# Tanveer81/ReVisionLLM

Measured on AMD Instinct MI355X. Metric: video-segments/sec (whole node), stage-2 100-seg recursion, Vicuna-7B, higher is better.
Workload: dtype fp16

## Files before the change

### revisionllm_amd/csrc/gemm_pp.hip

```cpp
#include <algorithm>
#include <atomic>
#include <type_traits>

#include "kernels.h"

#ifndef PP_ABL
#define PP_ABL 0
#endif
#if PP_ABL & 32
__device__ __attribute__((visibility("default"))) unsigned long long pp_stamp_buf[256 * 2 * 9];
__device__ __attribute__((visibility("default"))) unsigned long long pp_stamp_ext[3 * 256 * 4];
#endif

namespace {

typedef const __attribute__((address_space(1))) void* gptr_t;
typedef __attribute__((address_space(3))) void* lptr_t;
__device__ __forceinline__ void glds16(const void* g, void* l) { __builtin_amdgcn_global_load_lds((gptr_t)g, (lptr_t)l, 16, 0, 0); }
__device__ __forceinline__ float silu(float x) { return rv_silu(x); }

constexpr int PBM = 256, PBN = 256, PBK = 64;
constexpr int UNIT = 128 * 128;
constexpr int PP_LDS = 10 * UNIT;

// ... 24 lines not shown
#pragma unroll
    for (int i = 0; i < 2; ++i) {
        const int lr = (wave * 2 + i) * 8 + (lane >> 3);
        const int chunk = (lane & 7) ^ (lane >> 3);
        const int trow = (lr >> 6) * 128 + (lr & 63);
        int g0 = m0 + trow, g1 = m0 + trow + 64;
        g0 = g0 < M ? g0 : M - 1;
        g1 = g1 < M ? g1 : M - 1;
        s.a0[i] = (unsigned)(((int64_t)g0 * lda + chunk * 8) * 2);
        s.a1[i] = (unsigned)(((int64_t)g1 * lda + chunk * 8) * 2);
    }
    const int kfr = K >> 5;
    const int nb0 = ((PP_ABL & 16) ? 0 : (n0 >> 4)) + (wave >> 1) * NF + (wave & 1);
#pragma unroll
    for (int ks = 0; ks < 2; ++ks) {
        s.w0[ks] = (unsigned)(((((int64_t)nb0 * kfr + ks) * 64 + lane) * 8) * 2);
        s.w1[ks] = (unsigned)(((((int64_t)(nb0 + 2) * kfr + ks) * 64 + lane) * 8) * 2);
    }
    if constexpr (NF == 3) {
        const int nb1 = (n0 >> 4) + (wave >> 1) * NF + 2;
        s.w1[0] = (unsigned)(((((int64_t)nb1 * kfr + (wave & 1)) * 64 + lane) * 8) * 2);
    }
}

template <int U, int NF>
__device__ __forceinline__ void issue_unit(const PpSrc& s, int k0, char* dst0, int wave) {
    char* dst = dst0 + wave * 2048;
    const char* ab = s.A + (int64_t)k0 * 2;
    const char* wb = s.W + (int64_t)k0 * 32;
    if constexpr (U == 0) {
        glds16(ab + s.a0[0], dst);
        glds16(ab + s.a0[1], dst + 1024);
    } else if constexpr (U == 3) {
        glds16(ab + s.a1[0], dst);
        glds16(ab + s.a1[1], dst + 1024);
    } else if constexpr (U == 1) {
        glds16(wb + s.w0[0], dst);
        glds16(wb + s.w0[1], dst + 1024);
    } else if constexpr (NF == 4) {
        glds16(wb + s.w1[0], dst);
        glds16(wb + s.w1[1], dst + 1024);
    } else {
        glds16(wb + s.w1[0], dst0 + wave * 1024);
    }
}

template <int N_>
__device__ __forceinline__ void wait_vm() {
    static_assert(N_ >= 0 && N_ <= 14, "extend the table");
    if constexpr (N_ == 14) asm volatile("s_waitcnt vmcnt(14)" ::: "memory");
    else if constexpr (N_ == 13) asm volatile("s_waitcnt vmcnt(13)" ::: "memory");
    else if constexpr (N_ == 12) asm volatile("s_waitcnt vmcnt(12)" ::: "memory");
    else if constexpr (N_ == 11) asm volatile("s_waitcnt vmcnt(11)" ::: "memory");
    else if constexpr (N_ == 10) asm volatile("s_waitcnt vmcnt(10)" ::: "memory");
    else if constexpr (N_ == 9) asm volatile("s_waitcnt vmcnt(9)" ::: "memory");
    else if constexpr (N_ == 8) asm volatile("s_waitcnt vmcnt(8)" ::: "memory");
    else if constexpr (N_ == 7) asm volatile("s_waitcnt vmcnt(7)" ::: "memory");
    else if constexpr (N_ == 6) asm volatile("s_waitcnt vmcnt(6)" ::: "memory");
    else if constexpr (N_ == 5) asm volatile("s_waitcnt vmcnt(5)" ::: "memory");
    else if constexpr (N_ == 4) asm volatile("s_waitcnt vmcnt(4)" ::: "memory");
    else if constexpr (N_ == 3) asm volatile("s_waitcnt vmcnt(3)" ::: "memory");
    else if constexpr (N_ == 2) asm volatile("s_waitcnt vmcnt(2)" ::: "memory");
    else if constexpr (N_ == 1) asm volatile("s_waitcnt vmcnt(1)" ::: "memory");
    else asm volatile("s_waitcnt vmcnt(0)" ::: "memory");
}

#ifndef PP_ISSUE_MID
#define PP_ISSUE_MID 0
#endif
#ifndef PP_PRIO_MODE
#define PP_PRIO_MODE 1
#endif
#define _PP_C ,
constexpr int PP_A_STAGE = 2 * UNIT, PP_W_BASE = 2 * PP_A_STAGE, PP_W_STAGE = 2 * UNIT;
typedef int pp_i32x8 __attribute__((ext_vector_type(8)));
__device__ __forceinline__ pp_i32x8 pp_cat(op16x8 lo, op16x8 hi) {
    typedef int i32x4_ __attribute__((ext_vector_type(4)));
    const i32x4_ a = __builtin_bit_cast(i32x4_, lo), b = __builtin_bit_cast(i32x4_, hi);
    return pp_i32x8{a[0], a[1], a[2], a[3], b[0], b[1], b[2], b[3]};
}
#ifndef PP_KSPLIT
#define PP_KSPLIT 1
#endif
#ifndef PP_EARLY
#define PP_EARLY 0
#endif
__device__ __forceinline__ void glds16_sv(const char* sbase, unsigned voff, char* lds_dst) {
    const unsigned l = (unsigned)(uintptr_t)(lptr_t)lds_dst;
    asm volatile("s_mov_b32 m0, %2\n\ts_nop 0\n\tglobal_load_lds_dwordx4 %0, %1" : : "v"(voff), "s"(sbase), "s"(l) : "memory");
}
template <int KIND>
__device__ __forceinline__ void issue_ks(const PpSrc& s, int kt, char* dst0, int wave) {
    char* dst = dst0 + wave * 2048;
    const char* ab = s.A + (int64_t)kt * (PBK * 2);
    const char* wb = s.W + (int64_t)kt * (PBK * 32);
    if constexpr (KIND == 0) {
        glds16_sv(ab, s.a0[0], dst);
        glds16_sv(ab, s.a0[1], dst + 1024);
    } else if constexpr (KIND == 1) {
        glds16_sv(ab, s.a1[0], dst);
        glds16_sv(ab, s.a1[1], dst + 1024);
    } else {
        glds16_sv(wb, s.w0[KIND - 2], dst);
        glds16_sv(wb, s.w1[KIND - 2], dst + 1024);
    }
}
__device__ __forceinline__ void ks_issue_prologue(const PpSrc& src, int kt0, int nks, char* smem, int wave) {
    issue_ks<2>(src, kt0, smem + 1 * UNIT, wave);
    issue_ks<0>(src, kt0, smem + 2 * UNIT, wave);
    issue_ks<3>(src, kt0, smem + 3 * UNIT, wave);
    issue_ks<1>(src, kt0, smem + 4 * UNIT, wave);
    if (nks > 1) {
        issue_ks<2>(src, kt0 + 1, smem + 5 * UNIT, wave);
        issue_ks<0>(src, kt0 + 1, smem + 6 * UNIT, wave);
        issue_ks<3>(src, kt0 + 1, smem + 7 * UNIT, wave);
        issue_ks<1>(src, kt0 + 1, smem + 8 * UNIT, wave);
        if (nks > 2) issue_ks<2>(src, kt0 + 2, smem + 9 * UNIT, wave);
    }
}
template <int DUMMY = 0>
__device__ __forceinline__ void pp_mainloop_ks(f32x4 (&acc)[4][8], const PpSrc& src, int kt0, int nks, char* smem, int wave, int lane, [[maybe_unused]] int kind = 1,
                                               bool pre = false) {
    const int wr = wave >> 2, wc = wave & 3;
    const int fr = lane & 15, kg = lane >> 4;
    const int a_rd = (wr * 64 + fr) * 128;
    const int a_c0 = ((kg ^ (fr & 7)) << 4), a_c1 = (((4 + kg) ^ (fr & 7)) << 4);
    const int w_rd = wc * 4096 + lane * 16;
    auto slot = [&](int ib, int k) { const int x = ib + k; return smem + (x >= 10 ? x - 10 : x) * UNIT; };
    op16x8 A0[4], A1[4], W0[4], W1[4];
    [[maybe_unused]] uint32_t st_sum[8] = {0, 0, 0, 0, 0, 0, 0, 0};
    [[maybe_unused]] uint64_t st_prev = 0;
#if PP_ABL & 32
#define PP_STAMP(i) { const uint64_t t_ = __builtin_readcyclecounter(); st_sum[i] += (uint32_t)(t_ - st_prev); st_prev = t_; }
#else
#define PP_STAMP(i)
#endif
#define KS_READ_A(DST, BASE, CH)                                                                            \
    if constexpr (!(PP_ABL & 2)) _Pragma("unroll") for (int f = 0; f < 4; ++f) DST[f] = *(const op16x8*)((BASE) + a_rd + f * 2048 + (CH));
#define KS_READ_W(DST, BASE)                                                                                \
    if constexpr (!(PP_ABL & 2)) _Pragma("unroll") for (int j = 0; j < 4; ++j) DST[j] = *(const op16x8*)((BASE) + w_rd + (j & 1) * 2048 + (j >> 1) * 1024);
#define KS_MFMA(WB, AB, MI0)                                                                                \
    if constexpr (!(PP_ABL & 8)) _Pragma("unroll") for (int j = 0; j < 4; ++j) _Pragma("unroll") for (int f = 0; f < 4; ++f) \
        acc[j][(MI0) + f] = rv_mfma16(WB[j], AB[f], acc[j][(MI0) + f]);
#define KS_SYNC_M(WAITN)                                   \
    if constexpr (grp == 1) { WAITN; }                     \
    __builtin_amdgcn_sched_barrier(0);                     \
    if constexpr (!(PP_ABL & 4)) __builtin_amdgcn_s_barrier(); \
    __builtin_amdgcn_sched_barrier(0);
#define KS_SYNC_C(WAITN)                                   \
    __builtin_amdgcn_sched_barrier(0);                     \
    if constexpr (grp == 0) { WAITN; }                     \
    __builtin_amdgcn_sched_barrier(0);                     \
    if constexpr (!(PP_ABL & 4)) __builtin_amdgcn_s_barrier(); \
    __builtin_amdgcn_sched_barrier(0);
    if constexpr (PP_ABL & 2) {
        asm volatile("" : "=v"(A0[0]), "=v"(A0[1]), "=v"(A0[2]), "=v"(A0[3]), "=v"(A1[0]), "=v"(A1[1]), "=v"(A1[2]), "=v"(A1[3]));
        asm volatile("" : "=v"(W0[0]), "=v"(W0[1]), "=v"(W0[2]), "=v"(W0[3]), "=v"(W1[0]), "=v"(W1[1]), "=v"(W1[2]), "=v"(W1[3]));
    }

#if PP_ABL & 32
    const uint64_t t_in = __builtin_readcyclecounter();
#endif
    if (!pre) ks_issue_prologue(src, kt0, nks, smem, wave);
    if (nks > 2) wait_vm<14>();
    else if (nks > 1) wait_vm<12>();
    else wait_vm<4>();
    __builtin_amdgcn_s_barrier();
    KS_READ_A(A0, smem + 2 * UNIT, a_c0)
    KS_READ_W(W0, smem + 1 * UNIT)
    if (nks > 2) wait_vm<12>();
    else if (nks > 1) wait_vm<10>();
    else wait_vm<2>();
// ... 251 lines not shown
        s.a[i] = (unsigned)(((int64_t)g * lda + (((lane & 7) ^ (lane >> 3)) * 8)) * 2);
        const int nb = (n0 >> 4) + wave * 4 + (i >> 1);
        s.w[i] = (unsigned)(((((int64_t)nb * kfr + (i & 1)) * 64 + lane) * 8) * 2);
    }
}
constexpr int PP4_TILE = 256 * 64 * 2;
template <int DUMMY = 0>
__device__ __forceinline__ void pp4_mainloop(f32x4 (&acc)[8][8], const Pp4Src& src, int kt0, int nks, char* smem, int wave, int lane) {
    const int wr = wave >> 1, wc = wave & 1;
    const int fr = lane & 15, kg = lane >> 4;
    const int a_rd = (wr * 128 + fr) * 128;
    const int a_c[2] = {((kg ^ (fr & 7)) << 4), (((4 + kg) ^ (fr & 7)) << 4)};
    const int w_rd = wc * 16384 + lane * 16;
    op16x8 fa[2][8], fw[2][8];
#define P4_A_STAGE(c) (smem + ((c) & 1) * PP4_TILE)
#define P4_W_STAGE(ws) (smem + (2 + (ws)) * PP4_TILE)
#define P4_ISSUE_A(KT, ST, i) glds16(src.A + (int64_t)(KT) * 128 + src.a[i], (ST) + (wave * 8 + (i)) * 1024)
#define P4_ISSUE_W(KT, ST, i) glds16(src.W + (int64_t)(KT) * 2048 + src.w[i], (ST) + (wave * 8 + (i)) * 1024)
#define P4_READ_A(B, ST, KS, f) fa[B][f] = *(const op16x8*)((ST) + a_rd + (f) * 2048 + a_c[KS])
#define P4_READ_W(B, ST, KS, j) fw[B][j] = *(const op16x8*)((ST) + w_rd + (j) * 2048 + (KS) * 1024)
#define P4_MFMA1(B, j, f) asm volatile(RV_MFMA16_ASM " %0, %1, %2, %0" : "+a"(acc[j][f]) : "v"(fw[B][j]), "v"(fa[B][f]));
#define P4_MFMA2(B, j, f) P4_MFMA1(B, j, f) P4_MFMA1(B, j, (f) + 1)
#define P4_PIN __builtin_amdgcn_sched_barrier(0);
    const int last = kt0 + nks - 1;
    auto kclamp = [&](int k) { return k < last ? k : last; };
#pragma unroll
    for (int i = 0; i < 8; ++i) P4_ISSUE_A(kt0, P4_A_STAGE(0), i);
#pragma unroll
    for (int i = 0; i < 8; ++i) P4_ISSUE_W(kt0, P4_W_STAGE(0), i);
#pragma unroll
    for (int i = 0; i < 8; ++i) P4_ISSUE_W(kclamp(kt0 + 1), P4_W_STAGE(1), i);
#pragma unroll
    for (int i = 0; i < 8; ++i) P4_ISSUE_A(kclamp(kt0 + 1), P4_A_STAGE(1), i);
#pragma unroll
    for (int i = 0; i < 8; ++i) P4_ISSUE_W(kclamp(kt0 + 2), P4_W_STAGE(2), i);
    asm volatile("s_waitcnt vmcnt(24)" ::: "memory");
    __builtin_amdgcn_s_barrier();
#pragma unroll
    for (int f = 0; f < 8; ++f) { P4_READ_A(0, P4_A_STAGE(0), 0, f); P4_READ_W(0, P4_W_STAGE(0), 0, f); }
    int ws = 0;
    for (int c = 0; c < nks; ++c) {
        char* a_cur = P4_A_STAGE(c);
        char* a_nxt = P4_A_STAGE(c + 1);
        char* w_cur = P4_W_STAGE(ws);
        const int ws1 = ws == 2 ? 0 : ws + 1;
        char* w_nxt = P4_W_STAGE(ws1);
        const int ka = kclamp(kt0 + c + 2), kw = kclamp(kt0 + c + 3);
        P4_PIN
#pragma unroll
        for (int j = 0; j < 8; ++j) {
            P4_MFMA2(0, j, 0) P4_PIN
            P4_READ_A(1, a_cur, 1, j); P4_MFMA2(0, j, 2) P4_PIN
            P4_READ_W(1, w_cur, 1, j); P4_MFMA2(0, j, 4) P4_PIN
            P4_MFMA2(0, j, 6) P4_PIN
        }
        asm volatile("s_waitcnt vmcnt(8)" ::: "memory");
        __builtin_amdgcn_s_barrier();
        P4_PIN
#pragma unroll
        for (int j = 0; j < 8; ++j) {
            P4_MFMA2(1, j, 0) P4_PIN
            if (j < 4) { P4_READ_A(0, a_nxt, 0, 2 * j); P4_ISSUE_A(ka, a_cur, 2 * j); } else { P4_READ_W(0, w_nxt, 0, 2 * (j - 4)); P4_ISSUE_W(kw, w_cur, 2 * (j - 4)); }
            P4_MFMA2(1, j, 2) P4_PIN
            if (j < 4) { P4_READ_A(0, a_nxt, 0, 2 * j + 1); } else { P4_READ_W(0, w_nxt, 0, 2 * (j - 4) + 1); }
            P4_MFMA2(1, j, 4) P4_PIN
            if (j < 4) { P4_ISSUE_A(ka, a_cur, 2 * j + 1); } else { P4_ISSUE_W(kw, w_cur, 2 * (j - 4) + 1); }
            P4_MFMA2(1, j, 6) P4_PIN
        }
        ws = ws1;
    }
    asm volatile("s_waitcnt vmcnt(0) lgkmcnt(0)\n s_nop 15\n s_nop 15" ::: "memory");
    __builtin_amdgcn_s_barrier();
#undef P4_A_STAGE
#undef P4_W_STAGE
#undef P4_ISSUE_A
#undef P4_ISSUE_W
#undef P4_READ_A
#undef P4_READ_W
#undef P4_MFMA1
#undef P4_MFMA2
#undef P4_PIN
}

template <int NFR>
__device__ __forceinline__ void pp_rope_row_store(const f32x4 (&v)[NFR], const QkvRope& qr, const QkvRow& row, int sec, int head, int slab0, int kg) {
    const int p0 = slab0 + kg * 4;
    if constexpr ((RS_PROBE_K_ & 256) != 0) { if (sec == 2) return; }
    if constexpr ((RS_PROBE_K_ & 512) != 0) { if (sec == 1) return; }
    if constexpr ((RS_PROBE_K_ & 1024) != 0) { if (sec == 0) return; }
    if (sec == 2) {
        for (int bb = row.b0; bb < row.b1; ++bb) {
            op16_t* dst = (op16_t*)qr.vtc + ((int64_t)bb * qr.H + head) * 128 * qr.Smax + rv_vt_index(p0, row.pos);
#pragma unroll
            for (int ni = 0; ni < NFR; ++ni)
#pragma unroll
                for (int e = 0; e < 4; ++e) dst[(ni * 16 + e) * 8] = f32_to_op16(v[ni][e]);
        }
        return;
    }
    u32x2 o[NFR];
#pragma unroll
    for (int ni = 0; ni < NFR; ++ni) {
        const f32x4 t = *(const f32x4*)(row.cs + (p0 + ni * 16));
        const float a0 = __fmaf_rn(v[ni][0], t[0], -__fmul_rn(v[ni][1], t[1])), b0 = __fmaf_rn(v[ni][1], t[0], __fmul_rn(v[ni][0], t[1]));
        const float a1 = __fmaf_rn(v[ni][2], t[2], -__fmul_rn(v[ni][3], t[3])), b1 = __fmaf_rn(v[ni][3], t[2], __fmul_rn(v[ni][2], t[3]));
        o[ni] = pack_op16x4(f32x4{a0, b0, a1, b1});
    }
    if (sec == 0) {
        op16_t* dst = (op16_t*)qr.q16 + (int64_t)row.mrow * (qr.H * 128) + head * 128 + p0;
#pragma unroll
        for (int ni = 0; ni < NFR; ++ni) *(u32x2*)(dst + ni * 16) = o[ni];
    } else {
        for (int bb = row.b0; bb < row.b1; ++bb) {
            op16_t* dst = (op16_t*)qr.kc + (((int64_t)bb * qr.H + head) * qr.Smax + row.pos) * 128 + p0;
#pragma unroll
            for (int ni = 0; ni < NFR; ++ni) *(u32x2*)(dst + ni * 16) = o[ni];
        }
    }
}
template <int F8>
__device__ __forceinline__ void pp_epilogue_rope_lds(const f32x4 (&acc)[4][8], int M, int m0, int n0, int wave, int lane, const QkvRope& qr, const PpScale& sc,
                                                     char* smem) {
    constexpr int RS = 144;
    constexpr int TILE = 128 * RS, WREG = TILE + 128 * 16;
    static_assert(8 * WREG <= PP_LDS, "eight private wave regions");
    char* my = smem + wave * WREG;
    int4* info = (int4*)(my + TILE);
    const int wr = wave >> 2, wc = wave & 3, fr = lane & 15, kg = lane >> 4;
    const int D = qr.H * 128, nb = n0 + wc * 64;
    const int sec = __builtin_amdgcn_readfirstlane(nb / D), hd0 = nb - sec * D, head = hd0 >> 7, slab0 = hd0 & 127;
    const int mbase = m0 + wr * 128;
#pragma unroll
    for (int hh = 0; hh < 2; ++hh) {
        const int r = lane + 64 * hh, m = mbase + r;
        const QkvRow row = qkv_rope_row(qr, m < M ? m : M - 1);
        info[r] = (m < M && row.b1 > row.b0) ? int4{row.pos, row.b0, row.b1, row.mrow} : int4{-1, 0, 0, 0};
    }
    asm volatile("s_waitcnt lgkmcnt(0)" ::: "memory");
    int posv[8];
#pragma unroll
    for (int mi = 0; mi < 8; ++mi) {
        const int p_ = ((const int*)(info + mi * 16 + fr))[0];
        posv[mi] = p_ >= 0 ? p_ : qr.cs_pos0;
    }
    uint32_t sat = 0;
    if (sec == 2) {
#pragma unroll
        for (int ni = 0; ni < 4; ++ni)
#pragma unroll
            for (int mi = 0; mi < 8; ++mi) {
                f32x4 v = acc[ni][mi];
                if constexpr (F8) v = pp_scaled(sc, mbase + mi * 16 + fr, nb + ni * 16 + kg * 4, v);
                *(u32x2*)(my + (mi * 16 + fr) * RS + (ni * 16 + kg * 4) * 2) = u32x2{pack_op16x2_m(v[0], v[1], sat), pack_op16x2_m(v[2], v[3], sat)};
            }
    } else {
        const float* cs0 = qr.cs + (slab0 + kg * 4) - (int64_t)qr.cs_pos0 * 128;
        f32x4 tc[8], tn[8];
#pragma unroll
        for (int mi = 0; mi < 8; ++mi) tc[mi] = *(const f32x4*)(cs0 + (int64_t)posv[mi] * 128);
#pragma unroll
        for (int ni = 0; ni < 4; ++ni) {
            if (ni < 3) {
#pragma unroll
                for (int mi = 0; mi < 8; ++mi) tn[mi] = *(const f32x4*)(cs0 + (int64_t)posv[mi] * 128 + (ni + 1) * 16);
            }
#pragma unroll
            for (int mi = 0; mi < 8; ++mi) {
                f32x4 v = acc[ni][mi];
                if constexpr (F8) v = pp_scaled(sc, mbase + mi * 16 + fr, nb + ni * 16 + kg * 4, v);
                const f32x4 t = tc[mi];
                const float a0 = __fmaf_rn(v[0], t[0], -__fmul_rn(v[1], t[1])), b0 = __fmaf_rn(v[1], t[0], __fmul_rn(v[0], t[1]));
                const float a1 = __fmaf_rn(v[2], t[2], -__fmul_rn(v[3], t[3])), b1 = __fmaf_rn(v[3], t[2], __fmul_rn(v[2], t[3]));
                *(u32x2*)(my + (mi * 16 + fr) * RS + (ni * 16 + kg * 4) * 2) = u32x2{pack_op16x2_m(a0, b0, sat), pack_op16x2_m(a1, b1, sat)};
            }
#pragma unroll
            for (int mi = 0; mi < 8; ++mi) tc[mi] = tn[mi];
        }
    }
    rv_note_saturation(sat);
    if constexpr ((RS_PROBE_K_ & 2048) != 0) return;
    asm volatile("s_waitcnt lgkmcnt(0)" ::: "memory");
    if (sec < 2) {
        const int rl = lane >> 3, ch = lane & 7;
#pragma unroll 4
        for (int it = 0; it < 16; ++it) {
            const int r = it * 8 + rl;
            const int4 ri = info[r];
            if (ri.x < 0) continue;
            const u32x4 val = *(const u32x4*)(my + r * RS + ch * 16);
            if (sec == 0) {
                *(u32x4*)((op16_t*)qr.q16 + (int64_t)ri.w * D + head * 128 + slab0 + ch * 8) = val;
            } else {
                for (int bb = ri.y; bb < ri.z; ++bb)
                    *(u32x4*)((op16_t*)qr.kc + (((int64_t)bb * qr.H + head) * qr.Smax + ri.x) * 128 + slab0 + ch * 8) = val;
            }
        }
        return;
    }
    const int64_t vrow = (int64_t)128 * qr.Smax;
    for (int r = 0; r < 128;) {
        const int4 a = info[r];
        const int pos = __builtin_amdgcn_readfirstlane(a.x), b0 = __builtin_amdgcn_readfirstlane(a.y), b1 = __builtin_amdgcn_readfirstlane(a.z);
        if (pos < 0) { ++r; continue; }
        bool full = (pos & 7) == 0 && r + 7 < 128;
        if (full) {
            const int4 z = info[r + 7];
            full = __builtin_amdgcn_readfirstlane(z.x) == pos + 7 && __builtin_amdgcn_readfirstlane(z.y) == b0 && __builtin_amdgcn_readfirstlane(z.z) == b1;
        }
        const char* col = my + r * RS + lane * 2;
        if (full) {
            u32x4 w;
#pragma unroll
            for (int j = 0; j < 4; ++j)
                w[j] = (uint32_t)*(const uint16_t*)(col + (2 * j) * RS) | ((uint32_t)*(const uint16_t*)(col + (2 * j + 1) * RS) << 16);
            for (int bb = b0; bb < b1; ++bb)
                *(u32x4*)((op16_t*)qr.vtc + ((int64_t)bb * qr.H + head) * vrow + rv_vt_index(slab0 + lane, pos)) = w;
            r += 8;
        } else {
            const op16_t val = *(const op16_t*)col;
            for (int bb = b0; bb < b1; ++bb) ((op16_t*)qr.vtc)[((int64_t)bb * qr.H + head) * vrow + rv_vt_index(slab0 + lane, pos)] = val;
            ++r;
        }
    }
}

template <int OUT_BF16, int ACT, int ROPE, int NF, int F8 = 0>
__device__ __forceinline__ void pp_epilogue(const f32x4 (&acc_in)[NF][8], const float* __restrict__ bias, const float* res, int64_t ldr,
                                            void* Cv, int64_t ldc, int M, int m0, int n0, int wave, int lane, const QkvRope& qr,
                                            const PpScale& sc = PpScale{nullptr, nullptr}) {
    static_assert(NF == 4 || ACT != RV_ACT_SILU_MUL, "the gated epilogue pairs fragments: 256-column panels only");
    constexpr int WN = NF * 16;
    const int wr = wave >> 2, wc = wave & 3;
    const int fr = lane & 15, kg = lane >> 4;
#pragma unroll
    for (int mi = 0; mi < 8; ++mi) {
        const int m = m0 + wr * 128 + mi * 16 + fr;
        if (m >= M) continue;
        f32x4 acc[NF][1];
#pragma unroll
        for (int ni = 0; ni < NF; ++ni) acc[ni][0] = F8 ? pp_scaled(sc, m, n0 + wc * WN + ni * 16 + kg * 4, acc_in[ni][mi]) : acc_in[ni][mi];
        if constexpr (ROPE && NF == 4) {
            const int D = qr.H * 128, nb = n0 + wc * WN;
            const int sec = __builtin_amdgcn_readfirstlane(nb / D), hd0 = nb - sec * D;
            const QkvRow row = qkv_rope_row(qr, m);
            if (row.b1 > row.b0) {
                f32x4 v[4];
#pragma unroll
                for (int ni = 0; ni < 4; ++ni) v[ni] = acc[ni][0];
                pp_rope_row_store<4>(v, qr, row, sec, hd0 >> 7, hd0 & 127, kg);
            }
        } else if constexpr (ROPE) {
#pragma unroll
            for (int ni = 0; ni < NF; ++ni) qkv_rope_store(qr, m, n0 + wc * WN + ni * 16 + kg * 4, acc[ni][0]);
        } else if (ACT == RV_ACT_SILU_MUL) {
#pragma unroll
            for (int ni = 0; ni + 1 < NF; ni += 2) {
                const int n = n0 + wc * WN + ni * 16;
                const int no = (n >> 1) + kg * 4;
                float v[4];
#pragma unroll
                for (int r = 0; r < 4; ++r) v[r] = silu(acc[ni][0][r]) * acc[ni + 1][0][r];
                if constexpr ((RS_PROBE_K_ & 32768) != 0) {
                    const u32x2 o_ = pack_op16x4(v);
                    asm volatile("" ::"v"(o_[0]), "v"(o_[1]));
                    continue;
                }
                if constexpr ((PP_ABL & 64) != 0) {
                    asm volatile("" ::"v"(v[0]), "v"(v[1]), "v"(v[2]), "v"(v[3]));
                    continue;
                }
                if (OUT_BF16) *(u32x2*)((op16_t*)Cv + (int64_t)m * ldc + no) = pack_op16x4(v);
                else *(f32x4*)((float*)Cv + (int64_t)m * ldc + no) = f32x4{v[0], v[1], v[2], v[3]};
            }
        } else {
#pragma unroll
            for (int ni = 0; ni < NF; ++ni) {
                const int n = n0 + wc * WN + ni * 16 + kg * 4;
                f32x4 v = acc[ni][0];
                if (bias) v += *(const f32x4*)(bias + n);
                if (ACT == RV_ACT_RELU || ACT == RV_ACT_QUICK_GELU) {
#pragma unroll
                    for (int r = 0; r < 4; ++r) v[r] = rv_act_apply<ACT>(v[r]);
                }
                if (res) v += rv_residual4(res, ldr, m, n);
                if constexpr ((PP_ABL & 64) != 0) {
                    asm volatile("" ::"v"(v));
                    continue;
                }
                if (OUT_BF16) *(u32x2*)((op16_t*)Cv + (int64_t)m * ldc + n) = pack_op16x4(v);
                else *(f32x4*)((float*)Cv + (int64_t)m * ldc + n) = v;
            }
        }
    }
}

template <int OUT_BF16, int ACT, int ROPE>
__device__ __forceinline__ void pp4_epilogue(const f32x4 (&acc)[8][8], const float* __restrict__ bias, const float* res, int64_t ldr, void* Cv,
                                             int64_t ldc, int M, int m0, int n0, int wave, int lane, const QkvRope& qr) {
    const int wr = wave >> 1, wc = wave & 1;
    const int fr = lane & 15, kg = lane >> 4;
    if constexpr (ROPE) {
        const int D = qr.H * 128, nb = n0 + wc * 128;
        const int sec = __builtin_amdgcn_readfirstlane(nb / D), hd0 = nb - sec * D, head = hd0 >> 7;
// ... 100 lines not shown
    if (m >= M) return;
    const int nf = n0 + (W4 ? (w & 1) * 128 : (w & 3) * 64) + nip * 32;
    if constexpr (F8) {
        v0 = pp_scaled(sc, m, nf + kg * 4, v0);
        v1 = pp_scaled(sc, m, nf + 16 + kg * 4, v1);
    }
    if constexpr (ROPE) {
        qkv_rope_store(qr, m, nf + kg * 4, v0);
        qkv_rope_store(qr, m, nf + 16 + kg * 4, v1);
    } else if (ACT == RV_ACT_SILU_MUL) {
        const int no = (nf >> 1) + kg * 4;
        float v[4];
#pragma unroll
        for (int r = 0; r < 4; ++r) v[r] = silu(v0[r]) * v1[r];
        if (OUT_BF16) *(u32x2*)((op16_t*)Cv + (int64_t)m * ldc + no) = pack_op16x4(v);
        else *(f32x4*)((float*)Cv + (int64_t)m * ldc + no) = f32x4{v[0], v[1], v[2], v[3]};
    } else {
#pragma unroll
        for (int e = 0; e < 2; ++e) {
            const int n = nf + e * 16 + kg * 4;
            f32x4 v = e ? v1 : v0;
            if (bias) v += *(const f32x4*)(bias + n);
            if (ACT == RV_ACT_RELU || ACT == RV_ACT_QUICK_GELU) {
#pragma unroll
                for (int r = 0; r < 4; ++r) v[r] = rv_act_apply<ACT>(v[r]);
            }
            if (res) v += rv_residual4(res, ldr, m, n);
            if (OUT_BF16) *(u32x2*)((op16_t*)Cv + (int64_t)m * ldc + n) = pack_op16x4(v);
            else *(f32x4*)((float*)Cv + (int64_t)m * ldc + n) = v;
        }
    }
}

template <int C, int OUT_BF16, int ACT, int ROPE, int F8 = 0, int W4 = 0>
__device__ __forceinline__ void pp_reduce_share(f32x4* partial, const int* ids, int c, int j, int wave, int lane,
                                                const float* __restrict__ bias, const float* res, int64_t ldr, void* Cv, int64_t ldc,
                                                int M, int m0, int n0, const QkvRope& qr, const PpScale& sc = PpScale{nullptr, nullptr},
                                                float poison = 0.f) {
    constexpr int NW = W4 ? 4 : 8;
    constexpr int UPW = C <= 4 ? (128 + NW * C - 1) / (NW * C) : 1;
    const int per_pass = NW * UPW;
    for (int q0 = 0; j + q0 * c < 128; q0 += per_pass) {
        f32x4 s[UPW][2];
#pragma unroll
        for (int u = 0; u < UPW; ++u) s[u][0] = s[u][1] = f32x4{poison, poison, poison, poison};
        for (int base = 0; base < c; base += C) {
            f32x4 v[UPW][C][2];
#pragma unroll
            for (int i = 0; i < C; ++i) {
                const bool have = base + i < c;
                const __amdgpu_buffer_rsrc_t r = pp_slot_rsrc(partial, __builtin_amdgcn_readfirstlane(ids[have ? base + i : 0]));
#pragma unroll
                for (int u = 0; u < UPW; ++u) {
                    const int x = j + (q0 + wave + NW * u) * c;
                    const unsigned fragx = W4 ? (unsigned)((x >> 5) * 64 + (x & 3) * 16 + ((x >> 2) & 7)) : (unsigned)((x >> 4) * 32 + (x & 1) * 16 + ((x >> 1) & 7));
                    const unsigned off = (have && x < 128) ? (fragx * 64 + lane) * 16 : PP_OOB;
                    v[u][i][0] = ld_sc1(r, off);
                    v[u][i][1] = ld_sc1(r, off == PP_OOB ? PP_OOB : off + 8 * 1024);
                }
            }
#pragma unroll
            for (int u = 0; u < UPW; ++u)
#pragma unroll
                for (int i = 0; i < C; ++i) {
                    s[u][0] += v[u][i][0];
                    s[u][1] += v[u][i][1];
                }
        }
#pragma unroll
        for (int u = 0; u < UPW; ++u) {
            const int x = j + (q0 + wave + NW * u) * c;
            if (x < 128) {
                if constexpr (W4) pp_epilogue_unit<OUT_BF16, ACT, ROPE, F8, 1>(s[u][0], s[u][1], x >> 5, (x >> 2) & 7, x & 3, bias, res, ldr, Cv, ldc, M, m0, n0, lane, qr, sc);
                else pp_epilogue_unit<OUT_BF16, ACT, ROPE, F8>(s[u][0], s[u][1], x >> 4, (x >> 1) & 7, x & 1, bias, res, ldr, Cv, ldc, M, m0, n0, lane, qr, sc);
            }
        }
    }
}

template <int OUT_BF16, int ACT, int ROPE, int NF, int F8, int W4>
__device__ __forceinline__ void pp_sk_body(const op16_t* __restrict__ A, int64_t lda, const op16_t* __restrict__ Wp,
                                           const float* __restrict__ bias, const float* res, int64_t ldr, void* Cv,
                                           int64_t ldc, int M, int N, int K, int tiles_m, int TS, int nk, int dp_panels,
                                           int total_units, f32x4* partial, int* flags, int* status, int epoch, const QkvRope& qr,
                                           const PpScale& sc, int PGx, int tiles_n) {
    static_assert(!W4 || (NF == 4 && !F8), "the four-wave form: bf16 operands, 256-column panels");
    extern __shared__ __attribute__((aligned(16))) char smem[];
    const int tid = threadIdx.x, lane = tid & 63;
    const int wave = __builtin_amdgcn_readfirstlane(tid >> 6);
    const int xcd = blockIdx.x & 7, slot = blockIdx.x >> 3;
    const int teams_per_x = (gridDim.x >> 3) / TS;
    const int PG = PGx & 255, MHS = PGx >> 8;
    const int team = xcd * teams_per_x + slot / TS, tsl = slot % TS, tm = tsl % tiles_m, pgi = tsl / tiles_m;
    const int T = 8 * teams_per_x;
    if (pgi >= PG || slot >= teams_per_x * TS) return;
    auto unit_m0 = [&](int v) { return ((v & ((1 << MHS) - 1)) * tiles_m + tm) * PBM; };
    auto unit_panel = [&](int v) { return (v >> MHS) * PG + pgi; };
    auto ub = [&](int t) { return (int)((int64_t)t * total_units / T); };
    const int u_begin = ub(team), u_end = ub(team + 1);
    int shared_panel[2] = {-1, -1};

    const int whole_rounds = dp_panels / T;
    struct Item {
        int panel, ks0, nks, sk_panel, n0, m0;
        bool ok;
    };
    int u_ = u_begin, r_ = 0;
    auto next_item = [&]() {
        Item it{0, 0, 0, -1, 0, 0, false};
        for (;;) {
            it.sk_panel = -1;
            if (u_ < u_end) {
                it.sk_panel = u_ / nk;
                it.ks0 = u_ - it.sk_panel * nk;
                it.nks = min(nk - it.ks0, u_end - u_);
                it.panel = dp_panels + it.sk_panel;
                u_ += it.nks;
            } else if (r_ < whole_rounds) {
                it.panel = r_ * T + team;
                it.ks0 = 0;
                it.nks = nk;
                ++r_;
            } else {
                return it;
            }
            const int tpanel = unit_panel(it.panel);
            if (tpanel >= tiles_n) continue;
            it.n0 = tpanel * (NF * 64);
            it.m0 = unit_m0(it.panel);
            it.ok = true;
            return it;
        }
    };
    constexpr bool KS_LOOP = !W4 && NF == 4 && !F8 && (PP_KSPLIT & (ROPE ? 2 : 1)) != 0;
    constexpr bool EARLY = KS_LOOP && ROPE != 2 && PP_EARLY;
    [[maybe_unused]] PpSrc src_pre;
    [[maybe_unused]] bool pre = false;
    for (Item it = next_item(); it.ok;) {
        [[maybe_unused]] const int panel = it.panel;
        const int ks0 = it.ks0, nks = it.nks, sk_panel = it.sk_panel, n0 = it.n0;
        int m0 = it.m0;
        asm volatile("" : "+s"(m0));
        constexpr int NFW = W4 ? 8 : NF;
        f32x4 acc[NFW][8];
#pragma unroll
        for (int i = 0; i < NFW; ++i)
#pragma unroll
            for (int j = 0; j < 8; ++j) acc[i][j] = f32x4{0.f, 0.f, 0.f, 0.f};
#if PP_ABL & 32
        const uint64_t t_ml = __builtin_readcyclecounter();
#endif
        if constexpr (W4) {
            Pp4Src src;
            pp4_sources(src, A, lda, Wp, M, K, m0, n0, wave, lane);
            pp4_mainloop(acc, src, ks0, nks, smem, wave, lane);
        } else {
            PpSrc src;
            if (EARLY && pre) src = src_pre;
            else pp_sources<NF>(src, A, lda, Wp, M, K, m0, n0, wave, lane);
            pp_mainloop<NF, F8, (PP_KSPLIT & (ROPE ? 2 : 1)) != 0>(acc, src, ks0, nks, smem, wave, lane, ROPE ? 2 : ACT == RV_ACT_SILU_MUL ? 0 : 1, EARLY && pre);
        }
        it = next_item();
        pre = false;
        if constexpr (EARLY) {
            if (ks0 == 0 && nks == nk && it.ok) {
                pp_sources<NF>(src_pre, A, lda, Wp, M, K, it.m0, it.n0, wave, lane);
                ks_issue_prologue(src_pre, it.ks0, it.nks, smem, wave);
                pre = true;
            }
        }
#if PP_ABL & 32
        if (tid == 0 && blockIdx.x < 256) atomicAdd(&pp_stamp_ext[((ROPE ? 2 : ACT == RV_ACT_SILU_MUL ? 0 : 1) * 256 + blockIdx.x) * 4 + 1], (unsigned long long)(__builtin_readcyclecounter() - t_ml));
#endif

#if PP_ABL & 32
        const uint64_t t_ep = __builtin_readcyclecounter();
#define PP_EP_STAMP if (tid == 0 && blockIdx.x < 256) { atomicAdd(&pp_stamp_ext[((ROPE ? 2 : ACT == RV_ACT_SILU_MUL ? 0 : 1) * 256 + blockIdx.x) * 4 + 2], (unsigned long long)(__builtin_readcyclecounter() - t_ep)); atomicAdd(&pp_stamp_ext[((ROPE ? 2 : ACT == RV_ACT_SILU_MUL ? 0 : 1) * 256 + blockIdx.x) * 4 + 3], 1ull); }
#else
#define PP_EP_STAMP
#endif
        if (ks0 == 0 && nks == nk) {
            if constexpr (W4) pp4_epilogue<OUT_BF16, ACT, ROPE>(acc, bias, res, ldr, Cv, ldc, M, m0, n0, wave, lane, qr);
            else if constexpr (ROPE == 2 && NF == 4) {
                pp_epilogue_rope_lds<F8>(acc, M, m0, n0, wave, lane, qr, sc, smem);
                __syncthreads();
            } else pp_epilogue<OUT_BF16, ACT, ROPE, NF, F8>(acc, bias, res, ldr, Cv, ldc, M, m0, n0, wave, lane, qr, sc);
            PP_EP_STAMP
            continue;
        }
        if constexpr (NF == 4) {
            const int ps = ks0 == 0 ? 1 : 0, id = (team * TS + tsl) * 2 + ps;
            shared_panel[ps] = sk_panel;
            const __amdgpu_buffer_rsrc_t pr = pp_slot_rsrc(partial, id);
            const unsigned off = (wave * (NFW * 8) * 64 + lane) * 16;
#pragma unroll
            for (int ni = 0; ni < NFW; ++ni)
#pragma unroll
                for (int mi = 0; mi < 8; ++mi) st_sc1(pr, off + (ni * 8 + mi) * 1024, acc[ni][mi]);
            asm volatile("s_waitcnt vmcnt(0)" ::: "memory");
            __syncthreads();
            if (tid == 0) __hip_atomic_store(flags + id, epoch, __ATOMIC_RELAXED, __HIP_MEMORY_SCOPE_AGENT);
        }
    }
    if constexpr (NF != 4) return;

    int* ids = (int*)smem;
    for (int ps = 0; ps < 2; ++ps) {
        const int panel = shared_panel[ps];
        if (panel < 0) continue;
        const int lo = panel * nk, hi = lo + nk;
        int t0 = team, t1 = team;
        while (t0 > 0 && ub(t0) > lo) --t0;
        while (t1 + 1 < T && ub(t1 + 1) < hi) ++t1;
        __syncthreads();
        int c = 0, j = 0;
        for (int t = t0; t <= t1; ++t) {
            if (ub(t) == ub(t + 1)) continue;
            if (t == team) j = c;
            if (tid == 0) ids[c] = (t * TS + tsl) * 2 + (ub(t) <= lo ? 1 : 0);
            ++c;
        }
        if (tid == 0) {
            int gave_up = 0;
            for (int i = 0; i < c; ++i) {
                unsigned spins = 0;
                while (__hip_atomic_load(flags + ids[i], __ATOMIC_RELAXED, __HIP_MEMORY_SCOPE_AGENT) != epoch) {
                    __builtin_amdgcn_s_sleep(2);
                    if (++spins > (1u << 24)) {
                        *status = 1;
                        gave_up = 1;
                        break;
                    }
                }
            }
            ids[1024] = gave_up;
        }
        __syncthreads();
        const float poison = ids[1024] ? __int_as_float(0x7fc00000) : 0.f;
        const int m0 = unit_m0(dp_panels + panel), n0 = unit_panel(dp_panels + panel) * PBN;
        if (c == 2) pp_reduce_share<2, OUT_BF16, ACT, ROPE, F8, W4>(partial, ids, c, j, wave, lane, bias, res, ldr, Cv, ldc, M, m0, n0, qr, sc, poison);
        else if (c == 3) pp_reduce_share<3, OUT_BF16, ACT, ROPE, F8, W4>(partial, ids, c, j, wave, lane, bias, res, ldr, Cv, ldc, M, m0, n0, qr, sc, poison);
        else if (c == 4) pp_reduce_share<4, OUT_BF16, ACT, ROPE, F8, W4>(partial, ids, c, j, wave, lane, bias, res, ldr, Cv, ldc, M, m0, n0, qr, sc, poison);
        else pp_reduce_share<8, OUT_BF16, ACT, ROPE, F8, W4>(partial, ids, c, j, wave, lane, bias, res, ldr, Cv, ldc, M, m0, n0, qr, sc, poison);
    }
}

template <int OUT_BF16, int ACT, int ROPE, int NF, int F8 = 0>
__global__ __launch_bounds__(512) void gemm_pp_sk(const op16_t* __restrict__ A, int64_t lda, const op16_t* __restrict__ Wp,
                                                  const float* __restrict__ bias, const float* res, int64_t ldr, void* Cv,
                                                  int64_t ldc, int M, int N, int K, int tiles_m, int TS, int nk, int dp_panels,
                                                  int total_units, f32x4* partial, int* flags, int* status, int epoch, QkvRope qr,
                                                  PpScale sc, int PG, int tiles_n) {
    pp_sk_body<OUT_BF16, ACT, ROPE, NF, F8, 0>(A, lda, Wp, bias, res, ldr, Cv, ldc, M, N, K, tiles_m, TS, nk, dp_panels, total_units, partial, flags,
                                               status, epoch, qr, sc, PG, tiles_n);
}
template <int OUT_BF16, int ACT, int ROPE>
__global__ __launch_bounds__(256) __attribute__((amdgpu_waves_per_eu(1, 1))) void gemm_pp4_sk(
    const op16_t* __restrict__ A, int64_t lda, const op16_t* __restrict__ Wp, const float* __restrict__ bias, const float* res, int64_t ldr,
    void* Cv, int64_t ldc, int M, int N, int K, int tiles_m, int TS, int nk, int dp_panels, int total_units, f32x4* partial, int* flags,
    int* status, int epoch, QkvRope qr, PpScale sc, int PG, int tiles_n) {
    pp_sk_body<OUT_BF16, ACT, ROPE, 4, 0, 1>(A, lda, Wp, bias, res, ldr, Cv, ldc, M, N, K, tiles_m, TS, nk, dp_panels, total_units, partial, flags,
                                             status, epoch, qr, sc, PG, tiles_n);
}

int pp_device_cus() {
    static int n = 0;
    if (n == 0) {
        int dev = 0;
        (void)hipGetDevice(&dev);
        if (hipDeviceGetAttribute(&n, hipDeviceAttributeMultiprocessorCount, dev) != hipSuccess || n <= 0) n = 256;
    }
    return n;
}
int pp_num_cus() {
    const int n = pp_device_cus();
    const int want = rv_cur_opts().gemm_cus & ~7;
    return (want > 0 && want <= n) ? want : n;
}

template <typename Kern>
int reserve_lds(Kern k, std::atomic<uint64_t>& done) {
    int dev = 0;
    (void)hipGetDevice(&dev);
    const uint64_t bit = 1ull << (dev & 63);
    if (!(done.load(std::memory_order_relaxed) & bit)) {
        if (hipFuncSetAttribute((const void*)k, hipFuncAttributeMaxDynamicSharedMemorySize, PP_LDS) != hipSuccess) {
            rv_set_error("gemm_pp: cannot reserve %d bytes of LDS", PP_LDS);
            return RV_ERR_HIP;
// ... 235 lines not shown
```

Before: 6560.

## Load rope epilogue args late from kernarg and precompute V-transpose run flags

The RoPE LDS epilogue now reloads the QkvRope and scale fields straight from the kernarg segment after the main loop, instead of keeping them live in SGPRs through the MFMA loop. This is meant to reduce scalar register pressure in the main loop. The V-section check for whether an 8-row run is contiguous is now computed per lane ahead of time into the info slot, replacing serial readfirstlane comparisons. The multi-batch K/V stores use pointer increments instead of recomputing the full index each iteration. It also adds an m0 clobber to the inline asm and a separate KSPLIT bit for non-fused rope paths, which adds a risk of reading kernarg offsets wrongly if the struct layout diverges.

```diff
diff --git a/revisionllm_amd/csrc/gemm_pp.hip b/revisionllm_amd/csrc/gemm_pp.hip
--- a/revisionllm_amd/csrc/gemm_pp.hip
+++ b/revisionllm_amd/csrc/gemm_pp.hip
@@ -130,12 +130,17 @@
 #ifndef PP_KSPLIT
 #define PP_KSPLIT 1
 #endif
+template <int ROPE>
+constexpr bool pp_ksplit_on() { return (PP_KSPLIT & (ROPE == 2 ? 2 : ROPE ? 4 : 1)) != 0; }
 #ifndef PP_EARLY
 #define PP_EARLY 0
 #endif
 __device__ __forceinline__ void glds16_sv(const char* sbase, unsigned voff, char* lds_dst) {
     const unsigned l = (unsigned)(uintptr_t)(lptr_t)lds_dst;
-    asm volatile("s_mov_b32 m0, %2\n\ts_nop 0\n\tglobal_load_lds_dwordx4 %0, %1" : : "v"(voff), "s"(sbase), "s"(l) : "memory");
+#pragma clang diagnostic push
+#pragma clang diagnostic ignored "-Winline-asm"
+    asm volatile("s_mov_b32 m0, %2\n\ts_nop 0\n\tglobal_load_lds_dwordx4 %0, %1" : : "v"(voff), "s"(sbase), "s"(l) : "memory", "m0");
+#pragma clang diagnostic pop
 }
 template <int KIND>
 __device__ __forceinline__ void issue_ks(const PpSrc& s, int kt, char* dst0, int wave) {
@@ -553,6 +558,45 @@
 #undef P4_PIN
 }
 
+struct PpSkArgs {
+    const op16_t* A; int64_t lda; const op16_t* Wp; const float* bias; const float* res; int64_t ldr; void* Cv; int64_t ldc;
+    int M, N, K, tiles_m, TS, nk, dp_panels, total_units;
+    f32x4* partial; int* flags; int* status; int epoch;
+    QkvRope qr; PpScale sc; int PG, tiles_n;
+};
+static_assert(std::is_standard_layout<PpSkArgs>::value && std::is_standard_layout<QkvRope>::value, "offsetof");
+typedef const __attribute__((address_space(4))) char* kchar_t;
+typedef const __attribute__((address_space(4))) int* kint_t;
+template <typename F>
+__device__ __forceinline__ F pp_karg(kchar_t p, size_t off) { return *(const __attribute__((address_space(4))) F*)(p + off); }
+__device__ __forceinline__ void pp_late_args(QkvRope& q, kint_t& grow, PpScale& sc, int after) {
+    kchar_t p = (kchar_t)__builtin_amdgcn_kernarg_segment_ptr();
+    asm volatile("" : "+s"(p) : "s"(after));
+    kchar_t a = p + offsetof(PpSkArgs, qr);
+#define PP_LATE_F(NAME) q.NAME = pp_karg<decltype(q.NAME)>(a, offsetof(QkvRope, NAME));
+    PP_LATE_F(cs) PP_LATE_F(q16) PP_LATE_F(kc) PP_LATE_F(vtc) PP_LATE_F(B) PP_LATE_F(S) PP_LATE_F(P0) PP_LATE_F(pos0) PP_LATE_F(cs_pos0) PP_LATE_F(H) PP_LATE_F(Smax)
+    PP_LATE_F(G) PP_LATE_F(Mg) PP_LATE_F(ng) PP_LATE_F(gt)
+#undef PP_LATE_F
+    grow = (kint_t)(a + offsetof(QkvRope, grow));
+    sc.a = pp_karg<const float*>(p, offsetof(PpSkArgs, sc) + offsetof(PpScale, a));
+    sc.w = pp_karg<const float*>(p, offsetof(PpSkArgs, sc) + offsetof(PpScale, w));
+}
+__device__ __forceinline__ QkvRow pp_late_row(const QkvRope& q, kint_t grow, int m) {
+    QkvRow r;
+    r.mrow = m;
+    int goff = 0, b, mt = m;
+    bool prefix = false;
+    int B = q.B, P0 = q.P0, S = q.S, pos0 = q.pos0;
+    if (q.ng) { const QkvGroup e = qkv_rope_group(q, mt); B = e.B; P0 = pos0 = e.P0; S = e.S; goff = e.row; }
+    else if (q.G > 1) { const int gi = m / q.Mg; mt = m - gi * q.Mg; goff = grow[gi]; }
+    if (mt < P0) { b = 0; r.pos = mt; prefix = true; }
+    else { const int rr = mt - P0; b = rr / S; r.pos = pos0 + (rr - b * S); }
+    r.cs = nullptr;
+    r.b0 = (prefix ? 0 : b) + goff;
+    r.b1 = (prefix ? B : b + 1) + goff;
+    return r;
+}
+
 template <int NFR>
 __device__ __forceinline__ void pp_rope_row_store(const f32x4 (&v)[NFR], const QkvRope& qr, const QkvRow& row, int sec, int head, int slab0, int kg) {
     const int p0 = slab0 + kg * 4;
@@ -590,8 +634,8 @@
     }
 }
 template <int F8>
-__device__ __forceinline__ void pp_epilogue_rope_lds(const f32x4 (&acc)[4][8], int M, int m0, int n0, int wave, int lane, const QkvRope& qr, const PpScale& sc,
-                                                     char* smem) {
+__device__ __forceinline__ void pp_epilogue_rope_lds(const f32x4 (&acc)[4][8], int M, int m0, int n0, int wave, int lane, const QkvRope& qr, kint_t grow,
+                                                     const PpScale& sc, char* smem) {
     constexpr int RS = 144;
     constexpr int TILE = 128 * RS, WREG = TILE + 128 * 16;
     static_assert(8 * WREG <= PP_LDS, "eight private wave regions");
@@ -604,10 +648,19 @@
 #pragma unroll
     for (int hh = 0; hh < 2; ++hh) {
         const int r = lane + 64 * hh, m = mbase + r;
-        const QkvRow row = qkv_rope_row(qr, m < M ? m : M - 1);
+        const QkvRow row = pp_late_row(qr, grow, m < M ? m : M - 1);
         info[r] = (m < M && row.b1 > row.b0) ? int4{row.pos, row.b0, row.b1, row.mrow} : int4{-1, 0, 0, 0};
     }
     asm volatile("s_waitcnt lgkmcnt(0)" ::: "memory");
+    if (sec == 2) {
+#pragma unroll
+        for (int hh = 0; hh < 2; ++hh) {
+            const int r = lane + 64 * hh;
+            const int4 a = info[r], z = info[r + 7 < 128 ? r + 7 : 127];
+            ((int*)(info + r))[3] = (a.x >= 0 && (a.x & 7) == 0 && r + 7 < 128 && z.x == a.x + 7 && z.y == a.y && z.z == a.z) ? 1 : 0;
+        }
+        asm volatile("s_waitcnt lgkmcnt(0)" ::: "memory");
+    }
     int posv[8];
 #pragma unroll
     for (int mi = 0; mi < 8; ++mi) {
@@ -662,34 +715,35 @@
             if (sec == 0) {
                 *(u32x4*)((op16_t*)qr.q16 + (int64_t)ri.w * D + head * 128 + slab0 + ch * 8) = val;
             } else {
-                for (int bb = ri.y; bb < ri.z; ++bb)
-                    *(u32x4*)((op16_t*)qr.kc + (((int64_t)bb * qr.H + head) * qr.Smax + ri.x) * 128 + slab0 + ch * 8) = val;
+                const int64_t krow = (int64_t)qr.H * qr.Smax * 128;
+                op16_t* dst = (op16_t*)qr.kc + (((int64_t)ri.y * qr.H + head) * qr.Smax + ri.x) * 128 + slab0 + ch * 8;
+                *(u32x4*)dst = val;
+                for (int bb = ri.y + 1; bb < ri.z; ++bb) *(u32x4*)(dst += krow) = val;
             }
         }
         return;
     }
     const int64_t vrow = (int64_t)128 * qr.Smax;
+    const int64_t brow = (int64_t)qr.H * vrow;
     for (int r = 0; r < 128;) {
         const int4 a = info[r];
         const int pos = __builtin_amdgcn_readfirstlane(a.x), b0 = __builtin_amdgcn_readfirstlane(a.y), b1 = __builtin_amdgcn_readfirstlane(a.z);
         if (pos < 0) { ++r; continue; }
-        bool full = (pos & 7) == 0 && r + 7 < 128;
-        if (full) {
-            const int4 z = info[r + 7];
-            full = __builtin_amdgcn_readfirstlane(z.x) == pos + 7 && __builtin_amdgcn_readfirstlane(z.y) == b0 && __builtin_amdgcn_readfirstlane(z.z) == b1;
-        }
+        const bool full = __builtin_amdgcn_readfirstlane(a.w) != 0;
         const char* col = my + r * RS + lane * 2;
+        op16_t* dst = (op16_t*)qr.vtc + ((int64_t)b0 * qr.H + head) * vrow + rv_vt_index(slab0 + lane, pos);
         if (full) {
             u32x4 w;
 #pragma unroll
             for (int j = 0; j < 4; ++j)
                 w[j] = (uint32_t)*(const uint16_t*)(col + (2 * j) * RS) | ((uint32_t)*(const uint16_t*)(col + (2 * j + 1) * RS) << 16);
-            for (int bb = b0; bb < b1; ++bb)
-                *(u32x4*)((op16_t*)qr.vtc + ((int64_t)bb * qr.H + head) * vrow + rv_vt_index(slab0 + lane, pos)) = w;
+            *(u32x4*)dst = w;
+            for (int bb = b0 + 1; bb < b1; ++bb) *(u32x4*)(dst += brow) = w;
             r += 8;
         } else {
             const op16_t val = *(const op16_t*)col;
-            for (int bb = b0; bb < b1; ++bb) ((op16_t*)qr.vtc)[((int64_t)bb * qr.H + head) * vrow + rv_vt_index(slab0 + lane, pos)] = val;
+            *dst = val;
+            for (int bb = b0 + 1; bb < b1; ++bb) *(dst += brow) = val;
             ++r;
         }
     }
@@ -956,8 +1010,8 @@
 __device__ __forceinline__ void pp_sk_body(const op16_t* __restrict__ A, int64_t lda, const op16_t* __restrict__ Wp,
                                            const float* __restrict__ bias, const float* res, int64_t ldr, void* Cv,
                                            int64_t ldc, int M, int N, int K, int tiles_m, int TS, int nk, int dp_panels,
-                                           int total_units, f32x4* partial, int* flags, int* status, int epoch, const QkvRope& qr,
-                                           const PpScale& sc, int PGx, int tiles_n) {
+                                           int total_units, f32x4* partial, int* flags, int* status, int epoch, const QkvRope& qr_in,
+                                           const PpScale& sc_in, int PGx, int tiles_n) {
     static_assert(!W4 || (NF == 4 && !F8), "the four-wave form: bf16 operands, 256-column panels");
     extern __shared__ __attribute__((aligned(16))) char smem[];
     const int tid = threadIdx.x, lane = tid & 63;
@@ -1006,7 +1060,7 @@
             return it;
         }
     };
-    constexpr bool KS_LOOP = !W4 && NF == 4 && !F8 && (PP_KSPLIT & (ROPE ? 2 : 1)) != 0;
+    constexpr bool KS_LOOP = !W4 && NF == 4 && !F8 && pp_ksplit_on<ROPE>();
     constexpr bool EARLY = KS_LOOP && ROPE != 2 && PP_EARLY;
     [[maybe_unused]] PpSrc src_pre;
     [[maybe_unused]] bool pre = false;
@@ -1032,7 +1086,7 @@
             PpSrc src;
             if (EARLY && pre) src = src_pre;
             else pp_sources<NF>(src, A, lda, Wp, M, K, m0, n0, wave, lane);
-            pp_mainloop<NF, F8, (PP_KSPLIT & (ROPE ? 2 : 1)) != 0>(acc, src, ks0, nks, smem, wave, lane, ROPE ? 2 : ACT == RV_ACT_SILU_MUL ? 0 : 1, EARLY && pre);
+            pp_mainloop<NF, F8, pp_ksplit_on<ROPE>()>(acc, src, ks0, nks, smem, wave, lane, ROPE ? 2 : ACT == RV_ACT_SILU_MUL ? 0 : 1, EARLY && pre);
         }
         it = next_item();
         pre = false;
@@ -1054,11 +1108,15 @@
 #define PP_EP_STAMP
 #endif
         if (ks0 == 0 && nks == nk) {
-            if constexpr (W4) pp4_epilogue<OUT_BF16, ACT, ROPE>(acc, bias, res, ldr, Cv, ldc, M, m0, n0, wave, lane, qr);
+            if constexpr (W4) pp4_epilogue<OUT_BF16, ACT, ROPE>(acc, bias, res, ldr, Cv, ldc, M, m0, n0, wave, lane, qr_in);
             else if constexpr (ROPE == 2 && NF == 4) {
-                pp_epilogue_rope_lds<F8>(acc, M, m0, n0, wave, lane, qr, sc, smem);
+                QkvRope qr_l;
+                PpScale sc_l;
+                kint_t grow_l;
+                pp_late_args(qr_l, grow_l, sc_l, m0);
+                pp_epilogue_rope_lds<F8>(acc, M, m0, n0, wave, lane, qr_l, grow_l, sc_l, smem);
                 __syncthreads();
-            } else pp_epilogue<OUT_BF16, ACT, ROPE, NF, F8>(acc, bias, res, ldr, Cv, ldc, M, m0, n0, wave, lane, qr, sc);
+            } else pp_epilogue<OUT_BF16, ACT, ROPE, NF, F8>(acc, bias, res, ldr, Cv, ldc, M, m0, n0, wave, lane, qr_in, sc_in);
             PP_EP_STAMP
             continue;
         }
@@ -1078,6 +1136,8 @@
     }
     if constexpr (NF != 4) return;
 
+    const QkvRope& qr = qr_in;
+    const PpScale& sc = sc_in;
     int* ids = (int*)smem;
     for (int ps = 0; ps < 2; ++ps) {
         const int panel = shared_panel[ps];
```

New measurement: 6547. Within noise of the previous version (-0.2%).
